# EricssonResearch/Robust-Tracking-MPC-over-Lossy-Networks

Hardware: AMD Instinct MI355X
Metric: QP solves/sec (= MPC steps/sec) at batch (higher is better)
Workload: dtype f64

## Files before the change

robust-tracking-mpc-over-lossy-networks_amd/csrc/tmpc_kernels.hip:

```cpp
#ifdef TMPC_HOST_SIM
#include "hip_sim.hpp"
#else
#include <hip/hip_runtime.h>
#endif

#include <algorithm>
#include <cmath>
#include <cstdint>
#include <string>
#include <type_traits>
#include <utility>

#include "tmpc_device.hpp"
#include "tmpc_launch.hpp"
#include "tmpc_wave.hpp"
#include "tmpc_mc_step.hpp"
#include "tmpc_law.hpp"
#include "tmpc_law_wave.hpp"

namespace tmpc {

namespace {

using wv::WAVE;
using wv::fast_rcp;
using wv::readlane_d;
using wv::lanes_backsub_lane;
using wv::lanes_factor;
using wv::lanes_forward;
using wv::vmax;
using wv::vmax_abs;
using wv::vmin;
using wv::OpMax;
using wv::OpMin;
using wv::OpSum;

constexpr int RED_STRIDE = 68;
constexpr int ZERO_ROWS = 4;

#if defined(TMPC_HOST_SIM)
#define STAMP(p) do { } while (0)
#elif defined(TMPC_STAMPS)
#define STAMP(p) do { asm volatile("s_waitcnt vmcnt(0) lgkmcnt(0)" ::: "memory"); long long now_ = __builtin_amdgcn_s_memtime(); \
                      asm volatile("s_waitcnt lgkmcnt(0)" ::: "memory"); tph[p] += now_ - tlast; tlast = now_; } while (0)
#else
#define STAMP(p) do { asm volatile("; MARK " #p); } while (0)
#endif

#ifndef TMPC_FENCE_ALL
#define TMPC_FENCE_ALL 0
#endif
#ifdef TMPC_HOST_SIM
__device__ __forceinline__ void row_fence() {}
__device__ __forceinline__ void wave_lds_fence() { sim::wave_fence(); }
#else
__device__ __forceinline__ void row_fence() {
    asm volatile("" ::: "memory");
    __builtin_amdgcn_sched_barrier(0);
}
__device__ __forceinline__ void wave_lds_fence() { asm volatile("" ::: "memory"); }
#endif

__device__ __forceinline__ double rcp1(double x) {
    const double r = __builtin_amdgcn_rcp(x);
    return fma(fma(-x, r, 1.0), r, r);
}

__device__ __forceinline__ double wave_sum(double v) { return wv::wave_reduce<OpSum>(v); }
__device__ __forceinline__ double wave_min(double v) { return wv::wave_reduce<OpMin>(v); }
__device__ __forceinline__ double wave_max(double v) { return wv::wave_reduce<OpMax>(v); }

__device__ __forceinline__ int fresh(int v) {
#ifdef TMPC_HOST_SIM
    asm volatile("" : "+r"(v));
#else
    asm volatile("" : "+v"(v));
#endif
    return v;
}

template <int N, class F>
__device__ __forceinline__ void static_for(F &&f) {
    [&]<int... I>(std::integer_sequence<int, I...>) { (f(std::integral_constant<int, I>{}), ...); }(std::make_integer_sequence<int, N>{});
}

template <class SH, int CNT>
__device__ __forceinline__ void wave_sums_to_lds(const double (&acc)[CNT], double *red, double *out, int lane) {
    static_assert(RED_STRIDE == wv::RED_STRIDE, "one tile layout");
    wv::swap_reduce_to_lds<CNT, SH::RR>(acc, red, out, lane);
}

template <class SH, int OFF, int CNT, int TOT>
__device__ __forceinline__ void wave_sums_part(const double (&acc)[TOT], double *red, double *out, int lane) {
    static_assert(OFF + CNT <= TOT, "part of the array");
    double part[CNT];
#pragma unroll
    for (int i = 0; i < CNT; ++i) part[i] = acc[OFF + i];
    wave_sums_to_lds<SH, CNT>(part, red, out, lane);
}
template <class SH, int CNT, int SPLIT>
__device__ __forceinline__ void wave_sums_to_lds2(const double (&acc)[CNT], double *red, double *out0, double *out1, int lane) {
    wv::swap_reduce_to_lds_at<CNT, SH::RR>(acc, red, [out0, out1](int e) { return e < SPLIT ? out0 + e : out1 + (e - SPLIT); }, lane);
}

template <class SH, int WPB>
constexpr bool sweep_b_one_round() { return SH::FD > 0 && SH::KC > 0 && !(WPB == 8 && SH::NV == 12); }

template <int NV>
__host__ __device__ constexpr int col_off(int j) { return j * NV - j * (j - 1) / 2; }

constexpr int tile_rows(int nv, int wpb) { return (wpb == 8 || nv > 24) ? 12 : 16; }

template <int NV_, int DP_, int DS_, int KC_, int CP_, int CS_, int RR_>
struct Shape {
    static constexpr int NV = NV_, DP = DP_, DS = DS_, KC = KC_, CP = CP_, CS = CS_, RR = RR_;
    static constexpr int KCA = KC_ > 0 ? KC_ : 1;
    static constexpr int FD = DP_ + DS_, FC = CP_ + CS_;
    static constexpr int NDP = FD * WAVE, NCCP = FC * WAVE;
    static constexpr int RS = 2 * DP_ + DS_ + 2 * CP_ + CS_;
    static constexpr bool SKIPS = NV_ == 11 && DP_ == 1 && DS_ == 0 && KC_ == 5 && CP_ == 4 && CS_ == 0;
    static constexpr int NT = NV_ * (NV_ + 1) / 2, KT = KC_ * (KC_ + 1) / 2;
    static constexpr int WCAP = NV_ <= 24 ? 24 : 28;
    static constexpr int odd_up(int v) { return v | 1; }
    static constexpr int LDH = odd_up(NV_);
    static constexpr int LDM = odd_up(NV_ + 1);
    static constexpr int LDW = odd_up(NV_), LDT = odd_up(WCAP);
    static constexpr int NB = (NV_ + 1 + 15) / 16;
    static constexpr int LDG = 16 * NB + 1;
    static constexpr int NTL = NB * (NB + 1) / 2;
    static constexpr int dbase(int kd) { return kd < DP_ ? 2 * kd : 2 * DP_ + (kd - DP_); }
    static constexpr int dsides(int kd) { return kd < DP_ ? 2 : 1; }
    static constexpr int cbase(int kc) { return 2 * DP_ + DS_ + (kc < CP_ ? 2 * kc : 2 * CP_ + (kc - CP_)); }
    static constexpr int csides(int kc) { return kc < CP_ ? 2 : 1; }
};

template <class SH>
__device__ __forceinline__ void side_info(int i, bool &dense, int &fslot, double &sgn) {
    if (i < 2 * SH::DP) { dense = true; fslot = i >> 1; sgn = (i & 1) ? -1.0 : 1.0; return; }
    if (i < 2 * SH::DP + SH::DS) { dense = true; fslot = SH::DP + (i - 2 * SH::DP); sgn = 1.0; return; }
    const int j = i - (2 * SH::DP + SH::DS);
    dense = false;
    if (j < 2 * SH::CP) { fslot = j >> 1; sgn = (j & 1) ? -1.0 : 1.0; return; }
    fslot = SH::CP + (j - 2 * SH::CP);
    sgn = 1.0;
}

template <class SH>
struct WaveLds {
    static constexpr int RED = SH::RR * RED_STRIDE;
    static constexpr int POL = SH::WCAP * SH::LDW + SH::NV * SH::LDT + 4 * SH::WCAP;
    static constexpr int MFAC = SH::NV * SH::LDM;
    static constexpr int BIG = RED + MFAC > POL ? RED + MFAC : POL;
    static constexpr int SUMS = 2 * SH::NV + 8;
    static constexpr int CSUMS = SH::KT + 2 * SH::KC + 8;
    static constexpr int PMAT = SH::KCA * SH::NV;
    static constexpr int HROW = SH::RS * WAVE;
    static constexpr int VEC = 9 * SH::NV + 32;
    static constexpr int TOTAL = BIG + SUMS + CSUMS + PMAT + HROW + VEC;
    static constexpr int PARK_WORDS = SH::RS * WAVE + 2;
    static constexpr int IDLE_WORDS = 2 * ((BIG - POL) + SUMS + CSUMS + PMAT);
#ifdef TMPC_PARK_HBM
    static constexpr bool PARK_LDS = false;
#else
    static constexpr bool PARK_LDS = IDLE_WORDS >= PARK_WORDS;
#endif
    static_assert(RED >= 2 * SH::NDP, "(D, t) of the dense functionals share the transposition tile");
};

template <class SH>
__device__ __forceinline__ void coords_lds(const double *Psi, const double *vec, double *out, int lane) {
    if constexpr (SH::KC > 0) {
        const int a_ = lane < SH::KC ? lane : 0;
        double t = 0.0;
#pragma unroll
        for (int j = 0; j < SH::NV; ++j) t += Psi[a_ * SH::NV + j] * vec[j];
        if (lane < SH::KC) out[lane] = t;
    }
}

template <class SH, int KD>
__device__ __forceinline__ double dense_dot(const double *Gt, int grows, const double *v, int lane) {
    const double *g = Gt + min(lane + KD * WAVE, grows) * SH::LDG;
    double t0 = 0.0, t1 = 0.0;
#pragma unroll
    for (int j = 0; j + 1 < SH::NV; j += 2) { t0 += g[j] * v[j]; t1 += g[j + 1] * v[j + 1]; }
    if (SH::NV & 1) t0 += g[SH::NV - 1] * v[SH::NV - 1];
    return t0 + t1;
}
template <class SH, int KCS>
__device__ __forceinline__ double fact_dot(const double *Hct, const double *c, int lane) {
    const int r = lane + KCS * WAVE;
    double t = 0.0;
#pragma unroll
    for (int a = 0; a < SH::KC; ++a) t += Hct[a * SH::NCCP + r] * c[a];
    return t;
}

typedef double v4d __attribute__((ext_vector_type(4)));
template <class SH>
__device__ __forceinline__ void sweep_a_dense(const double *Gt, int nks, const double (&s)[SH::RS], const double (&lam)[SH::RS],
                                              const double *rpw, double (&rs)[SH::RS], double &gap_l,
                                              double *dtw, double *mt, double *gdr, int lane) {
    constexpr int NV = SH::NV, NB = SH::NB, LDG = SH::LDG, IT = NV / 16, CT = NV % 16;
    static_for<SH::FD>([&](auto kd_) {
        constexpr int kd = decltype(kd_)::value;
        double D = 0.0, t = 0.0;
#pragma unroll
        for (int sd = 0; sd < SH::dsides(kd); ++sd) {
            constexpr int base = SH::dbase(kd);
            const int i = base + sd;
            const double rsi = fast_rcp(s[i]);
            rs[i] = rsi;
            const double d = lam[i] * rsi;
            const double rpi = rpw[i * WAVE + lane];
            gap_l = fma(s[i], lam[i], gap_l);
            D += d;
            t = sd ? fma(-d, rpi, t) : fma(d, rpi, t);
        }
        dtw[2 * (kd * WAVE + lane)] = D;
        dtw[2 * (kd * WAVE + lane) + 1] = t;
    });
    wave_lds_fence();
    const int c = lane & 15, kq = lane >> 4;
    const double tmask = (c == CT) ? 1.0 : 0.0;
    constexpr int NACC = SH::NTL == 1 ? 2 : 1;
    v4d acc[NACC][SH::NTL];
#pragma unroll
    for (int h2 = 0; h2 < NACC; ++h2)
#pragma unroll
        for (int q = 0; q < SH::NTL; ++q) acc[h2][q] = v4d{0.0, 0.0, 0.0, 0.0};
    const double *dp = dtw + 2 * kq, *gp = Gt + kq * LDG + c;
    auto fetch = [&](double &Dk, double &tk, double (&g)[NB]) {
        Dk = dp[0];
        tk = dp[1];
#pragma unroll
        for (int blk = 0; blk < NB; ++blk) g[blk] = gp[16 * blk];
        dp += 8;
        gp += 4 * LDG;
    };
    auto multiply = [&](auto h_, double Dk, double tk, const double (&g)[NB]) {
        constexpr int h2 = decltype(h_)::value;
        double a[NB];
#pragma unroll
        for (int blk = 0; blk < NB; ++blk) a[blk] = Dk * g[blk];
        a[IT] = fma(tmask, tk, a[IT]);
#pragma unroll
        for (int I = 0; I < NB; ++I)
#pragma unroll
            for (int J = 0; J <= I; ++J)
                acc[h2][I * (I + 1) / 2 + J] = __builtin_amdgcn_mfma_f64_16x16x4f64(a[I], g[J], acc[h2][I * (I + 1) / 2 + J], 0, 0, 0);
    };
    {
        double D0, t0, g0[NB], D1, t1, g1[NB];
        fetch(D0, t0, g0);
        int ks = 0;
        for (; ks + 1 < nks; ks += 2) {
            fetch(D1, t1, g1);
            multiply(std::integral_constant<int, 0>{}, D0, t0, g0);
            fetch(D0, t0, g0);
            multiply(std::integral_constant<int, NACC - 1>{}, D1, t1, g1);
        }
        if (ks < nks) multiply(std::integral_constant<int, 0>{}, D0, t0, g0);
    }
    static_assert(WaveLds<SH>::RED >= 2 * (SH::NDP + 4), "look-ahead of the MFMA pass stays inside the transposition tile");
    double *mtk = mt + kq * SH::LDM + c;
#pragma unroll
    for (int I = 0; I < NB; ++I)
#pragma unroll
        for (int J = 0; J <= I; ++J)
#pragma unroll
            for (int reg = 0; reg < 4; ++reg) {
                const int row = 16 * I + kq + 4 * reg, col = 16 * J + c;
                double v = acc[0][I * (I + 1) / 2 + J][reg];
                if constexpr (NACC == 2) v += acc[1][I * (I + 1) / 2 + J][reg];
                if (row < NV && col < NV) {
                    mtk[(16 * I + 4 * reg) * SH::LDM + 16 * J] = v;
                    if (I != J) mt[col * SH::LDM + row] = v;
                }
                if (I == IT && row == NV && col < NV) gdr[col] = v;
            }
    wave_lds_fence();
}

template <class SH, int NCS>
__device__ __forceinline__ void sweep_a_factored(const double *Hct, const double (&s)[SH::RS], const double (&lam)[SH::RS],
                                                 const double *rpw, double (&rs)[SH::RS], double &gap_l, double obj_l,
                                                 double *red, double *csums, int lane) {
    constexpr int KC = SH::KC, KT = SH::KT, NCCP = SH::NCCP;
    double acc[KT + KC + 2];
    static_for<NCS>([&](auto kc_) {
        constexpr int kc = decltype(kc_)::value;
        const int r = lane + kc * WAVE;
        double hc[KC];
#pragma unroll
        for (int a = 0; a < KC; ++a) hc[a] = Hct[a * NCCP + r];
        double D = 0.0, t = 0.0;
#pragma unroll
        for (int sd = 0; sd < SH::csides(kc); ++sd) {
            constexpr int base = SH::cbase(kc);
            const int i = base + sd;
            const double rsi = fast_rcp(s[i]);
            rs[i] = rsi;
            const double d = lam[i] * rsi;
            const double rpi = rpw[i * WAVE + lane];
            gap_l = fma(s[i], lam[i], gap_l);
            D += d;
            t = sd ? fma(-d, rpi, t) : fma(d, rpi, t);
        }
#pragma unroll
        for (int a = 0; a < KC; ++a) {
            const double dg = D * hc[a];
#pragma unroll
            for (int b2 = a; b2 < KC; ++b2) acc[col_off<KC>(a) + b2 - a] = kc == 0 ? dg * hc[b2] : fma(dg, hc[b2], acc[col_off<KC>(a) + b2 - a]);
            acc[KT + a] = kc == 0 ? hc[a] * t : fma(hc[a], t, acc[KT + a]);
        }
    });
    acc[KT + KC] = gap_l;
    acc[KT + KC + 1] = obj_l;
    wave_sums_to_lds<SH, KT + KC + 2>(acc, red, csums, lane);
}

struct McNone {};
struct McStepArg {
    const McFused *rec;
    int t;
    uint8_t *gamma_out;
};
struct McLawArg {
    const McFused *rec;
    const LawLoop *law;
};
template <int FUSED> using McArg = std::conditional_t<FUSED == 1, const McFused *, std::conditional_t<FUSED == 2, McStepArg, McNone>>;
template <int FUSED> using McBodyArg = std::conditional_t<FUSED == 3, McLawArg, McArg<FUSED>>;
#if defined(TMPC_HOST_SIM)
typedef const McFused *McRecord;
__device__ __forceinline__ McRecord mc_record(const McFused *p) { return p; }
#else
typedef const __attribute__((address_space(4))) McFused *McRecord;
__device__ __forceinline__ McRecord mc_record(const McFused *p) {
    unsigned lo = static_cast<unsigned>(reinterpret_cast<uintptr_t>(p)), hi = static_cast<unsigned>(reinterpret_cast<uintptr_t>(p) >> 32);
    asm volatile("" : "+v"(lo), "+v"(hi));
    lo = __builtin_amdgcn_readfirstlane(lo);
    hi = __builtin_amdgcn_readfirstlane(hi);
    return (McRecord)((static_cast<uintptr_t>(hi) << 32) | lo);
}
#endif
#if defined(TMPC_HOST_SIM)
typedef const LawLoop *LawRecord;
__device__ __forceinline__ LawRecord law_record(const LawLoop *p) { return p; }
#else
typedef const __attribute__((address_space(4))) LawLoop *LawRecord;
__device__ __forceinline__ LawRecord law_record(const LawLoop *p) {
    unsigned lo = static_cast<unsigned>(reinterpret_cast<uintptr_t>(p)), hi = static_cast<unsigned>(reinterpret_cast<uintptr_t>(p) >> 32);
    asm volatile("" : "+v"(lo), "+v"(hi));
    lo = __builtin_amdgcn_readfirstlane(lo);
    hi = __builtin_amdgcn_readfirstlane(hi);
    return (LawRecord)((static_cast<uintptr_t>(hi) << 32) | lo);
}
#endif

template <int NV, int DP, int DS, int KC, int CP, int CS, int WPB, int FUSED, int NCS>
__device__ __forceinline__ void solve_body(
    const DeviceQP &qp, const int variant_id, const int64_t B,
    const double *__restrict__ x_k, const double *__restrict__ ref, const uint8_t *__restrict__ variant,
    double *__restrict__ u_nom, double *__restrict__ x_nom0, double *__restrict__ xu_ss,
    double *__restrict__ x_nom, int32_t *__restrict__ status, int32_t *__restrict__ iters,
    const int32_t *ws_in, int32_t *ws_out, unsigned long long *__restrict__ next_item,
    const McBodyArg<FUSED> mc) {
    using SH = Shape<NV, DP, DS, KC, CP, CS, tile_rows(NV, WPB)>;
    using WL = WaveLds<SH>;
    constexpr int RS = SH::RS, FD = SH::FD, FC = SH::FC, NDP = SH::NDP, NCCP = SH::NCCP, KT = SH::KT, WCAP = SH::WCAP, LDG = SH::LDG;
#ifdef TMPC_HOST_SIM
    double *smem = sim::lds<double>();
#else
    extern __shared__ __attribute__((aligned(16))) double smem[];
#endif
    double *wbase = smem;
    double *Hct = wbase + WPB * WL::TOTAL;
    double *Psi = Hct + KC * NCCP;
    double *Hs = Psi + KC * NV;
    double *Hinv = Hs + NV * SH::LDH;
    double *Gt = Hinv + NV * SH::LDH;
    const int grows = 4 * qp.nks;

    const int tid = threadIdx.x;
    const int lane_k = tid & (WAVE - 1);
    int lane = lane_k;
    const int wave = __builtin_amdgcn_readfirstlane(tid >> 6);
    const int nx = qp.nx, nu = qp.nu, N = qp.N, nc = qp.nc;
    constexpr int RSL = NCS == FC ? RS : SH::cbase(NCS);
    static_assert(NCS == FC || (SH::SKIPS && NCS == FC - 1), "the slot counts a layout of this shape can have");

    for (int i = tid; i < (grows + ZERO_ROWS) * LDG; i += blockDim.x) Gt[i] = (i < grows * LDG) ? qp.Gt[i] : 0.0;
    for (int i = tid; i < KC * NCCP; i += blockDim.x) Hct[i] = qp.Hct[i];
    for (int i = tid; i < KC * NV; i += blockDim.x) Psi[i] = qp.Psi[i];
    for (int i = tid; i < NV * NV; i += blockDim.x) { const int r_ = i / NV, c_ = i - r_ * NV; Hs[r_ * SH::LDH + c_] = qp.Hs[i]; Hinv[r_ * SH::LDH + c_] = qp.Hinv[i]; }
    __syncthreads();

    double *red = wbase + wave * WL::TOTAL;
    double *sums = red + WL::BIG;
    double *csums = sums + WL::SUMS;
    double *Pm = csums + WL::CSUMS;
    double *hw = Pm + WL::PMAT;
    double *vec = hw + WL::HROW;
    double *dtw = red;
    double *Mf = red + WL::RED;
    unsigned *park = reinterpret_cast<unsigned *>(red + WL::POL);
    double *qv = vec;
    double *zv = vec + NV;
    double *cgv = vec + 2 * NV;
    double *xin = vec + 3 * NV;
    double *tv = vec + 3 * NV + 32;
    double *uv = vec + 4 * NV + 32;
    double *dzav = vec + 5 * NV + 32;
    double *dzv = vec + 6 * NV + 32;
    double *czv = vec + 7 * NV + 32;
    double *cdzav = czv + 8;
    double *cdzv = czv + 16;

    const int vmask_k = static_cast<int>(qp.vmask[lane]);
    unsigned vmask = static_cast<unsigned>(vmask_k);
    auto valid = [&](int i) { return ((vmask >> i) & 1u) != 0u; };
#define TMPC_REFRESH() do { lane = fresh(lane_k); vmask = static_cast<unsigned>(fresh(vmask_k)); } while (0)

    const int64_t n_waves = static_cast<int64_t>(gridDim.x) * WPB;
    bool first_item = true;
    for (;;) {
        int64_t b;
        if (first_item) {
            b = B < n_waves ? static_cast<int64_t>(wave) * gridDim.x + blockIdx.x : static_cast<int64_t>(blockIdx.x) * WPB + wave;
            first_item = false;
        } else {
            unsigned long long drawn = ~0ull >> 2;
            if (lane_k == 0) {
                const unsigned long long seen = __hip_atomic_load(next_item, __ATOMIC_RELAXED, __HIP_MEMORY_SCOPE_AGENT);
                if (n_waves + static_cast<int64_t>(seen) < B) drawn = atomicAdd(next_item, 1ull);
            }
            b = n_waves + static_cast<int64_t>((static_cast<unsigned long long>(static_cast<unsigned>(__builtin_amdgcn_readfirstlane(static_cast<int>(drawn >> 32)))) << 32) |
                                               static_cast<unsigned>(__builtin_amdgcn_readfirstlane(static_cast<int>(drawn & 0xffffffffull))));
        }
        if (b >= B) break;
        if (variant != nullptr && variant[b] != variant_id) continue;
        if (variant == nullptr && variant_id != 0) continue;

        int n_steps = 1;
        if constexpr (FUSED == 1) n_steps = mc_record(mc)->T;
        if constexpr (FUSED == 3) n_steps = mc_record(mc.rec)->T;
        for (int t_mc = 0; t_mc < n_steps; ++t_mc) {
        TMPC_REFRESH();
        if constexpr (FUSED != 0) {
            McRecord mr;
            if constexpr (FUSED == 1) mr = mc_record(mc); else mr = mc_record(mc.rec);
            const double *xh = mr->st.x_hat, *rk = mr->st.ref_k;
            if (lane < nx) { xin[lane] = xh[b * nx + lane]; xin[nx + lane] = rk[b * nx + lane]; }
        } else {
            if (lane < nx) { xin[lane] = x_k[b * nx + lane]; xin[nx + lane] = ref[b * nx + lane]; }
        }
        wave_lds_fence();
        bool law_hit = false;
        if constexpr (FUSED == 3) {
            const LawRecord lr = law_record(mc.law);
            const int np = 2 * nx;
            const bool finite = __ballot(lane < np && !law_finite(xin[lane < np ? lane : 0])) == 0ull;
            int32_t *const region = lr->region;
            int tried = 0, chain_tests = 0, chain_end = LAW_HOP_NONE;
            const int max_hops = lr->max_hops;
            const int win = finite ? law_find(&lr->t[0], np, xin, __builtin_amdgcn_readfirstlane(region[b]), lr->max_tries, lane, tried, max_hops,
                                              chain_tests, chain_end)
                                   : -1;
            if (lane == 0 && max_hops > 0) law_count_hops(lr->hop_stats, chain_tests, chain_end);
            if (win >= 0) {
                const int ny0 = N * nu, ny = ny0 + 2 * nx + nu;
                const double *Kt = lr->t[0].K;
                for (int j = lane; j < ny; j += WAVE) {
                    const double s = law_row(Kt, win, ny, np, xin, j);
                    if (j < ny0) u_nom[b * ny0 + j] = s;
                    else if (j < ny0 + nx) x_nom0[b * nx + (j - ny0)] = s;
                    else xu_ss[b * (nx + nu) + (j - ny0 - nx)] = s;
                }
                if (lane == 0) {
                    status[b] = TMPC_STATUS_OPTIMAL;
                    iters[b] = 0;
                    if (qp.ticks) qp.ticks[b] = 0;
                    region[b] = win;
                    lr->hits[b] += 1;
                    lr->tries[b] += tried;
                    unsigned long long *th = lr->t[0].hits;
                    if (th) atomicAdd(th + win, 1ull);
                }
                law_hit = true;
            } else {
                unsigned long long *mn = lr->miss_n;
                unsigned long long slot = 0;
                if (lane == 0) {
                    region[b] = -1;
                    lr->tries[b] += tried;
                    slot = atomicAdd(mn, 1ull);
                }
                const unsigned lo = static_cast<unsigned>(__builtin_amdgcn_readfirstlane(static_cast<int>(slot & 0xffffffffull)));
                const unsigned hi = static_cast<unsigned>(__builtin_amdgcn_readfirstlane(static_cast<int>(slot >> 32)));
                const long long at = static_cast<long long>((static_cast<unsigned long long>(hi) << 32) | lo);
                if (at < lr->miss_cap) {
                    if (lane < np) lr->miss_p[at * np + lane] = xin[lane];
                    if (lane == 0) lr->miss_var[at] = 0;
                }
            }
        }
        if (!law_hit) {
        int st = TMPC_STATUS_MAX_ITER;
        int it_done = 0;
#ifdef TMPC_ITERS_TOTAL
        int n_reruns = 0, n_rounds = 0, amb_level = 0;
#endif
        const long long t_begin = qp.ticks ? static_cast<long long>(__builtin_amdgcn_s_memrealtime()) : 0;
#ifdef TMPC_STAMPS
        long long tph[16] = {0, 0, 0, 0, 0, 0, 0, 0, 0, 0, 0, 0, 0, 0, 0, 0};
        long long tlast = __builtin_amdgcn_s_memtime();
#endif
        bool infeasible_par = qp.always_infeasible != 0;
        for (int r = lane; r < qp.npar; r += WAVE) {
            double v = qp.gp0[r];
            for (int c = 0; c < nx; ++c) v += qp.Ep[r * nx + c] * xin[c];
            if (v < -1e-9 * (1.0 + fabs(qp.gp0[r]))) infeasible_par = true;
        }
        infeasible_par = __any(infeasible_par);

        if (lane < NV) {
            double v = 0.0;
            if (lane < qp.nv)
                for (int c = 0; c < nx; ++c) v += qp.F1s[lane * nx + c] * xin[c] + qp.F2s[lane * nx + c] * xin[nx + c];
            qv[lane] = v;
        }
        auto compute_h = [&]() {
            TMPC_REFRESH();
            double hv[RS];
            const double *__restrict__ E0 = qp.Esp + lane;
            constexpr size_t PL = static_cast<size_t>(RS) * WAVE;
            for (int c0 = 0; c0 < nx; c0 += 4) {
                double ev[4][RS];
#pragma unroll
                for (int u = 0; u < 4; ++u) {
                    const size_t cu = static_cast<size_t>(c0 + u < nx ? c0 + u : nx - 1);
#pragma unroll
                    for (int i = 0; i < RSL; ++i) ev[u][i] = E0[cu * PL + i * WAVE];
                }
                if (c0 == 0) {
#pragma unroll
                    for (int i = 0; i < RSL; ++i) hv[i] = qp.g0p[i * WAVE + lane];
                }
#pragma unroll
                for (int u = 0; u < 4; ++u) {
                    const double xc = c0 + u < nx ? xin[c0 + u] : 0.0;
#pragma unroll
                    for (int i = 0; i < RSL; ++i) hv[i] = fma(ev[u][i], xc, hv[i]);
                }
            }
            double hmax = 1.0;
#pragma unroll
            for (int i = 0; i < RSL; ++i) {
                if (valid(i)) hmax = fmax(hmax, fabs(hv[i]));
                hw[i * WAVE + lane] = hv[i];
            }
            wave_lds_fence();
            return hmax;
        };
        const double hn = wave_max(compute_h());
        double qn = 1.0;
#pragma unroll
        for (int j = 0; j < NV; ++j) qn = fmax(qn, fabs(qv[j]));
        qn = readlane_d(qn, 0);

        auto unconstrained_minimiser = [&]() {
            TMPC_REFRESH();
            if (lane < NV) {
                double v = 0.0;
#pragma unroll
                for (int j = 0; j < NV; ++j) v -= Hinv[lane * SH::LDH + j] * qv[j];
                zv[lane] = v;
            }
            wave_lds_fence();
            coords_lds<SH>(Psi, zv, czv, lane);
            wave_lds_fence();
        };
        auto raw_slacks = [&](double (&sl)[RS]) {
            TMPC_REFRESH();
            double smin = INFINITY;
            static_for<FD>([&](auto kd_) {
                constexpr int kd = decltype(kd_)::value;
                const double gz = dense_dot<SH, kd>(Gt, grows, zv, lane);
#pragma unroll
                for (int sd = 0; sd < SH::dsides(kd); ++sd) {
                    const int i = SH::dbase(kd) + sd;
                    sl[i] = hw[i * WAVE + lane] - (sd ? -gz : gz);
                    if (valid(i)) smin = vmin(smin, sl[i]);
                }
            });
            static_for<NCS>([&](auto kc_) {
                constexpr int kc = decltype(kc_)::value;
                const double gz = fact_dot<SH, kc>(Hct, czv, lane);
#pragma unroll
                for (int sd = 0; sd < SH::csides(kc); ++sd) {
                    const int i = SH::cbase(kc) + sd;
                    sl[i] = hw[i * WAVE + lane] - (sd ? -gz : gz);
                    if (valid(i)) smin = vmin(smin, sl[i]);
                }
            });
#pragma unroll
            for (int i = RSL; i < RS; ++i) sl[i] = 1.0;
            return smin;
        };

        double try_tol = qp.tol;
        const double ncd = static_cast<double>(nc);
        double rdn_last = 0.0;
        bool floor_tried = false;
        bool inW[RS];
        double yall[RS];
        int warm_m = 0;
        {
            unconstrained_minimiser();
            double sl[RS];
            const double smin = wave_min(raw_slacks(sl));
            if (infeasible_par) st = TMPC_STATUS_INFEASIBLE;
            else if (smin >= 0.0) st = TMPC_STATUS_OPTIMAL;
            if (ws_in != nullptr) warm_m = ws_in[b * WS_STRIDE];
        }
        STAMP(0);
        bool try_warm = warm_m > 0 && warm_m <= WCAP;
        int resume_it = -1;
        float *const save = qp.save ? qp.save + (static_cast<size_t>(blockIdx.x) * WPB + wave) * (2 * RS * WAVE) : nullptr;
        bool saved = false;
        bool h_valid = true;
        int ws_m = 0;
        if (st == TMPC_STATUS_MAX_ITER)
        for (;;) {
            bool want_polish = false;
            if (try_warm) {
#pragma unroll
                for (int i = 0; i < RS; ++i) { inW[i] = false; yall[i] = 0.0; }
                for (int k = 0; k < warm_m; ++k) {
                    const int gid = ws_in[b * WS_STRIDE + 1 + k];
#pragma unroll
                    for (int i = 0; i < RS; ++i) inW[i] = inW[i] || (gid == i * WAVE + lane && valid(i));
                }
                want_polish = true;
            } else {
                double s[RS], lam[RS], rs[RS];
                double *rpw = hw;
                double kappa = 1.0, rpn0 = 0.0;
                int it0 = 0;
                double mu_hand = 0.0;
                if (resume_it >= 0) {
                    if (!h_valid) { compute_h(); h_valid = true; }
                    coords_lds<SH>(Psi, zv, czv, lane);
                    wave_lds_fence();
                    (void)raw_slacks(s);
                    h_valid = false;
                    const double park_mu = WL::PARK_LDS ? *reinterpret_cast<const double *>(park + RS * WAVE) : 0.0;
                    const double park_thr = 1e3 * try_tol * hn;
#pragma unroll
                    for (int i = 0; i < RSL; ++i) {
                        const bool vl = valid(i);
                        const double raw = s[i];
                        double sv, lv;
                        if constexpr (WL::PARK_LDS) {
                            lv = fmax(static_cast<double>(__uint_as_float(park[i * WAVE + lane])), 1e-30);
                            sv = raw > park_thr ? raw : fmin(fmax(raw, park_mu * fast_rcp(lv)), park_thr);
                        } else {
                            sv = static_cast<double>(save[i * WAVE + lane]);
                            lv = static_cast<double>(save[(RS + i) * WAVE + lane]);
                            if (raw > 0.0 && fabs(sv - raw) <= 2.5e-7 * sv) sv = raw;
                        }
                        s[i] = vl ? sv : 1.0;
                        lam[i] = vl ? lv : 0.0;
                        const double rp0 = vl ? sv - raw : 0.0;
                        rpw[i * WAVE + lane] = rp0;
                        rpn0 = vmax_abs(rpn0, rp0);
                        rs[i] = 1.0;
                    }
#pragma unroll
                    for (int i = RSL; i < RS; ++i) { s[i] = 1.0; lam[i] = 0.0; rs[i] = 1.0; }
                    wave_lds_fence();
                    it0 = resume_it;
                    resume_it = -1;
                } else {
                    if (!h_valid) { compute_h(); h_valid = true; }
                    unconstrained_minimiser();
                    const double smin = wave_min(raw_slacks(s));
                    const double fl = 0.1 * fmax(-smin, 1.0);
                    h_valid = false;
                    double l1 = 0.0;
#pragma unroll
                    for (int i = 0; i < RSL; ++i) l1 = vmax(l1, valid(i) ? -s[i] * qp.cip[i * WAVE + lane] : 0.0);
                    l1 = wave_max(l1);
#ifdef TMPC_LAM0_ONE
                    const double lam0 = l1 < 0.0 ? 2.0 : 1.0;
#else
                    const double lam0 = fmin(fmax(sqrt(sqrt(l1)), 1.0), 1e3);
#endif
// ... 965 lines not shown
```

robust-tracking-mpc-over-lossy-networks_amd/csrc/tmpc_wave.hpp:

```cpp
#pragma once
#ifdef TMPC_HOST_SIM
#include "hip_sim.hpp"
#else
#include <hip/hip_runtime.h>
#endif

#include <utility>

namespace tmpc {
namespace wv {

constexpr int WAVE = 64;

__device__ __forceinline__ double fast_rcp(double x) {
    double r = __builtin_amdgcn_rcp(x);
    r = fma(fma(-x, r, 1.0), r, r);
    r = fma(fma(-x, r, 1.0), r, r);
    return r;
}

template <int CTRL>
__device__ __forceinline__ double dpp_mov_d(double v) {
    int lo = __double2loint(v), hi = __double2hiint(v);
    lo = __builtin_amdgcn_update_dpp(lo, lo, CTRL, 0xF, 0xF, false);
    hi = __builtin_amdgcn_update_dpp(hi, hi, CTRL, 0xF, 0xF, false);
    return __hiloint2double(hi, lo);
}
__device__ __forceinline__ double readlane_d(double v, int l) {
    const int lo = __builtin_amdgcn_readlane(__double2loint(v), l);
    const int hi = __builtin_amdgcn_readlane(__double2hiint(v), l);
    return __hiloint2double(hi, lo);
}
#ifdef TMPC_HOST_SIM
__device__ __forceinline__ double vmax(double a, double b) { return fmax(a, b); }
__device__ __forceinline__ double vmin(double a, double b) { return fmin(a, b); }
__device__ __forceinline__ double vmax_abs(double a, double b) { return fmax(a, fabs(b)); }
#else
__device__ __forceinline__ double vmax(double a, double b) {
    double r;
    asm("v_max_f64 %0, %1, %2" : "=v"(r) : "v"(a), "v"(b));
    return r;
}
__device__ __forceinline__ double vmin(double a, double b) {
    double r;
    asm("v_min_f64 %0, %1, %2" : "=v"(r) : "v"(a), "v"(b));
    return r;
}
__device__ __forceinline__ double vmax_abs(double a, double b) {
    double r;
    asm("v_max_f64 %0, %1, |%2|" : "=v"(r) : "v"(a), "v"(b));
    return r;
}
#endif
struct OpSum { __device__ __forceinline__ static double f(double a, double b) { return a + b; } };
struct OpMin { __device__ __forceinline__ static double f(double a, double b) { return vmin(a, b); } };
struct OpMax { __device__ __forceinline__ static double f(double a, double b) { return vmax(a, b); } };

template <class Op>
__device__ __forceinline__ double wave_reduce(double v) {
    v = Op::f(v, dpp_mov_d<0xB1>(v));
    v = Op::f(v, dpp_mov_d<0x4E>(v));
    v = Op::f(v, dpp_mov_d<0x141>(v));
    v = Op::f(v, dpp_mov_d<0x140>(v));
    const double r0 = readlane_d(v, 0), r1 = readlane_d(v, 16), r2 = readlane_d(v, 32), r3 = readlane_d(v, 48);
    return Op::f(Op::f(r0, r1), Op::f(r2, r3));
}

#ifdef TMPC_HOST_SIM
__device__ __forceinline__ void lds_fence() { sim::wave_fence(); }
#else
__device__ __forceinline__ void lds_fence() { asm volatile("" ::: "memory"); }
#endif

constexpr int RED_STRIDE = 68;
template <int CNT>
__device__ __forceinline__ void reduce_to_lds(const double (&acc)[CNT], double *red, double *out, int lane) {
    const int e = lane >> 2, qd = lane & 3;
    const int wcol = lane + (lane >> 4);
#pragma unroll
    for (int c0 = 0; c0 < CNT; c0 += 16) {
#pragma unroll
        for (int k = 0; k < 16; ++k)
            if (c0 + k < CNT) red[k * RED_STRIDE + wcol] = acc[c0 + k];
        lds_fence();
        double t = 0.0;
#pragma unroll
        for (int j = 0; j < 16; ++j) t += red[e * RED_STRIDE + qd * 17 + j];
        t += dpp_mov_d<0xB1>(t);
        t += dpp_mov_d<0x4E>(t);
        if (qd == 0 && c0 + e < CNT) out[c0 + e] = t;
        lds_fence();
    }
}

template <int HALF>
__device__ __forceinline__ void permlane_swap(int &x, int &y, int lane) {
    static_assert(HALF == 32 || HALF == 16, "v_permlane32_swap / v_permlane16_swap");
#ifdef TMPC_HOST_SIM
    const int xo = __builtin_amdgcn_readlane(x, lane ^ HALF), yo = __builtin_amdgcn_readlane(y, lane ^ HALF);
    const bool up = (lane & HALF) != 0;
    x = up ? yo : x;
    y = up ? y : xo;
#else
    (void)lane;
    if constexpr (HALF == 32) {
        const auto r = __builtin_amdgcn_permlane32_swap(x, y, false, false);
        x = static_cast<int>(r[0]);
        y = static_cast<int>(r[1]);
    } else {
        const auto r = __builtin_amdgcn_permlane16_swap(x, y, false, false);
        x = static_cast<int>(r[0]);
        y = static_cast<int>(r[1]);
    }
#endif
}
template <int HALF>
__device__ __forceinline__ double swap_add(double a, double b, int lane) {
    int alo = __double2loint(a), ahi = __double2hiint(a), blo = __double2loint(b), bhi = __double2hiint(b);
    permlane_swap<HALF>(alo, blo, lane);
    permlane_swap<HALF>(ahi, bhi, lane);
    return __hiloint2double(ahi, alo) + __hiloint2double(bhi, blo);
}

__device__ __forceinline__ void wave_sum2(double &a, double &b, int lane) {
    double v = swap_add<32>(a, b, lane);
    v += dpp_mov_d<0xB1>(v);
    v += dpp_mov_d<0x4E>(v);
    v += dpp_mov_d<0x141>(v);
    v += dpp_mov_d<0x140>(v);
    a = readlane_d(v, 0) + readlane_d(v, 16);
    b = readlane_d(v, 32) + readlane_d(v, 48);
}

template <int CNT, int RR, class OutAt>
__device__ __forceinline__ void swap_reduce_to_lds_at(const double (&acc)[CNT], double *red, OutAt &&out_at, int lane) {
    constexpr int H1 = (CNT + 1) / 2, H2 = (H1 + 1) / 2;
    double r1[H1];
#pragma unroll
    for (int c = 0; c < H1; ++c) r1[c] = swap_add<32>(acc[c], c + H1 < CNT ? acc[c + H1] : 0.0, lane);
    double r2[H2];
#pragma unroll
    for (int d = 0; d < H2; ++d) r2[d] = swap_add<16>(r1[d], d + H2 < H1 ? r1[d + H2] : 0.0, lane);
    auto entry = [](int d, int r) {
        const int e = d + (r & 1) * H2 + (r >> 1) * H1;
        return ((r & 1) && d + H2 >= H1) || e >= CNT ? -1 : e;
    };
    const int wcol = lane + (lane >> 4);
    const int k = lane >> 2, qd = lane & 3;
#pragma unroll
    for (int d0 = 0; d0 < H2; d0 += RR) {
#pragma unroll
        for (int d = 0; d < RR; ++d)
            if (d0 + d < H2) red[d * RED_STRIDE + wcol] = r2[d0 + d];
        lds_fence();
        constexpr int NR = RR < 16 ? RR : 16;
        const int kr = k < NR && d0 + k < H2 ? k : 0;
        double t4[4] = {0.0, 0.0, 0.0, 0.0};
#pragma unroll
        for (int j = 0; j < 16; ++j) t4[j & 3] += red[kr * RED_STRIDE + qd * 17 + j];
        const double t = (t4[0] + t4[1]) + (t4[2] + t4[3]);
        const int e = (k < NR && d0 + k < H2) ? entry(d0 + k, qd) : -1;
        if (e >= 0) *out_at(e) = t;
        lds_fence();
    }
}
template <int CNT, int RR>
__device__ __forceinline__ void swap_reduce_to_lds(const double (&acc)[CNT], double *red, double *out, int lane) {
    swap_reduce_to_lds_at<CNT, RR>(acc, red, [out](int e) { return out + e; }, lane);
}

template <int N>
__device__ __forceinline__ bool rows_factor(double (&row)[N], double &b, double &dinv, int lane) {
    bool ok = true;
#pragma unroll
    for (int k = 0; k < N; ++k) {
        const double pkk = readlane_d(row[k], k);
        ok = ok && (pkk > 0.0);
        const double pinv = fast_rcp(pkk);
        const double f = (lane > k) ? row[k] * pinv : 0.0;
#pragma unroll
        for (int j = k + 1; j < N; ++j) row[j] = fma(-f, readlane_d(row[j], k), row[j]);
        b = fma(-f, readlane_d(b, k), b);
        if (lane > k) row[k] = f;
        if (lane == k) dinv = pinv;
    }
    return ok;
}
template <int N>
__device__ __forceinline__ void rows_forward(const double (&row)[N], double &b, int lane) {
#pragma unroll
    for (int k = 0; k < N - 1; ++k) {
        const double f = (lane > k) ? row[k] : 0.0;
        b = fma(-f, readlane_d(b, k), b);
    }
}
template <int N>
__device__ __forceinline__ double rows_backsub_lane(const double (&row)[N], double b, double dinv, int lane) {
    double xl = 0.0;
#pragma unroll
    for (int i = N - 1; i >= 0; --i) {
        const double bi = b * dinv;
        const double xi = readlane_d(bi, i);
        xl = (lane == i) ? bi : xl;
        b = fma(-row[i], xi, b);
    }
    return xl;
}

template <int K>
__device__ __forceinline__ double row_bcast_d(double v) {
    return __builtin_amdgcn_mov_dpp(v, 0x150 + K, 0xF, 0xF, false);
}
template <int N, class F>
__device__ __forceinline__ void static_for_n(F &&f) {
    [&]<int... I>(std::integer_sequence<int, I...>) { (f(std::integral_constant<int, I>{}), ...); }(std::make_integer_sequence<int, N>{});
}
template <int K, int NOPS>
__device__ __forceinline__ void fmac_bcast(double &acc, double v, double m) {
#if defined(TMPC_HOST_SIM) || defined(TMPC_NO_DPP_FMAC)
    acc = fma(row_bcast_d<K>(v), m, acc);
#else
    if constexpr (NOPS > 0)
        asm volatile("s_nop %3\n\tv_fmac_f64_dpp %0, %1, %2 row_newbcast:%4 row_mask:0xf bank_mask:0xf"
                     : "+v"(acc) : "v"(v), "v"(m), "n"(NOPS - 1), "n"(K));
    else
        asm volatile("v_fmac_f64_dpp %0, %1, %2 row_newbcast:%3 row_mask:0xf bank_mask:0xf" : "+v"(acc) : "v"(v), "v"(m), "n"(K));
#endif
}
template <int K, int NOPS>
__device__ __forceinline__ double row_bcast_ordered(double v) {
#if defined(TMPC_HOST_SIM) || defined(TMPC_NO_DPP_FMAC)
    return row_bcast_d<K>(v);
#else
    double r;
    if constexpr (NOPS > 0)
        asm volatile("s_nop %2\n\tv_mov_b64_dpp %0, %1 row_newbcast:%3 row_mask:0xf bank_mask:0xf" : "=v"(r) : "v"(v), "n"(NOPS - 1), "n"(K));
    else
        asm volatile("v_mov_b64_dpp %0, %1 row_newbcast:%2 row_mask:0xf bank_mask:0xf" : "=v"(r) : "v"(v), "n"(K));
    return r;
#endif
}
__device__ __forceinline__ void pin(double &v) {
#if !defined(TMPC_HOST_SIM) && !defined(TMPC_NO_DPP_FMAC)
    asm volatile("" : "+v"(v));
#endif
}
template <int N>
__device__ __forceinline__ bool rows16_factor(double (&row)[N], double &b, double &dinv, int lane) {
    static_assert(N <= 16, "one matrix row per lane of a 16-lane DPP row");
    const int l16 = lane & 15;
    bool ok = true;
    pin(b);
    double pkk = row_bcast_ordered<0, 0>(row[0]);
    double pinv = fast_rcp(pkk);
    static_for_n<N>([&](auto k_) {
        constexpr int k = decltype(k_)::value;
        ok = ok && (pkk > 0.0);
        const double pinv_k = pinv;
        const double f = (l16 > k) ? row[k] * pinv_k : 0.0;
        const double nf = -f;
        constexpr int NU = N - 1 - k;
        static_for_n<(NU < 3 ? NU : 3)>([&](auto j_) {
            constexpr int j = k + 1 + decltype(j_)::value;
            fmac_bcast<k, 0>(row[j], row[j], nf);
        });
        if constexpr (NU < 3) fmac_bcast<k, 0>(b, b, nf);
        if constexpr (k + 1 < N) {
            pkk = row_bcast_ordered<k + 1, (NU == 1 ? 2 : 0)>(row[k + 1]);
            pinv = fast_rcp(pkk);
        }
        if constexpr (NU >= 3) {
            static_for_n<NU - 3>([&](auto j_) {
                constexpr int j = k + 4 + decltype(j_)::value;
                fmac_bcast<k, 0>(row[j], row[j], nf);
            });
            fmac_bcast<k, 0>(b, b, nf);
        }
        if (l16 > k) row[k] = f;
        if (l16 == k) dinv = pinv_k;
    });
    return __builtin_amdgcn_readfirstlane(static_cast<int>(ok)) != 0;
}
template <int N>
__device__ __forceinline__ void rows16_forward(const double (&row)[N], double &b, int lane) {
    const int l16 = lane & 15;
    static_for_n<N - 1>([&](auto k_) {
        constexpr int k = decltype(k_)::value;
        const double f = (l16 > k) ? row[k] : 0.0;
        b = fma(-f, row_bcast_d<k>(b), b);
    });
}
template <int N>
__device__ __forceinline__ double rows16_backsub_lane(const double (&row)[N], double b, double dinv, int lane) {
    const int l16 = lane & 15;
    double xl = 0.0;
    static_for_n<N>([&](auto r_) {
        constexpr int i = N - 1 - decltype(r_)::value;
        const double bi = b * dinv;
        const double xi = row_bcast_d<i>(bi);
        xl = (l16 == i) ? bi : xl;
        b = fma(-row[i], xi, b);
    });
    return xl;
}
template <int N, int LDM>
__device__ __forceinline__ bool rows32_factor_solve(double *Mf, const double *rhs, double *x, int lane) {
    static_assert(N > 16 && N <= 32, "two matrix rows per lane");
    const int l16 = lane & 15;
    const bool hasb = l16 + 16 < N;
    const int ib = hasb ? l16 + 16 : 0;
    double ra[N], rb[N];
#pragma unroll
    for (int j = 0; j < N; ++j) { ra[j] = Mf[l16 * LDM + j]; rb[j] = Mf[ib * LDM + j]; }
    double ba = rhs[l16], bb = hasb ? rhs[ib] : 0.0;
    double da = 1.0, db = 1.0;
    lds_fence();
    bool ok = true;
    pin(ba);
    pin(bb);
    static_for_n<N>([&](auto k_) {
        constexpr int k = decltype(k_)::value;
        constexpr bool inA = k < 16;
        constexpr int kl = k & 15;
        double pkk;
        if constexpr (inA) pkk = row_bcast_ordered<kl, (k >= N - 2 ? 2 : 0)>(ra[k]);
        else pkk = row_bcast_ordered<kl, (k >= N - 2 ? 2 : 0)>(rb[k]);
        ok = ok && (pkk > 0.0);
        const double pinv = fast_rcp(pkk);
        double nfa = 0.0;
        if constexpr (inA) nfa = (l16 > k) ? -ra[k] * pinv : 0.0;
        const double nfb = (hasb && l16 + 16 > k) ? -rb[k] * pinv : 0.0;
        static_for_n<N - 1 - k>([&](auto j_) {
            constexpr int j = k + 1 + decltype(j_)::value;
            if constexpr (inA) {
                fmac_bcast<kl, 0>(rb[j], ra[j], nfb);
                fmac_bcast<kl, 0>(ra[j], ra[j], nfa);
            } else {
                fmac_bcast<kl, 0>(rb[j], rb[j], nfb);
            }
        });
        if constexpr (inA) {
            fmac_bcast<kl, 0>(bb, ba, nfb);
            fmac_bcast<kl, 0>(ba, ba, nfa);
            if (l16 > k) ra[k] = -nfa;
            if (l16 == k) da = pinv;
        } else {
            fmac_bcast<kl, 0>(bb, bb, nfb);
            if (l16 == kl) db = pinv;
        }
        if (hasb && l16 + 16 > k) rb[k] = -nfb;
    });
    ok = __builtin_amdgcn_readfirstlane(static_cast<int>(ok)) != 0;
    if (!ok) return false;
    double xa = 0.0, xb = 0.0;
    static_for_n<N>([&](auto r_) {
        constexpr int i = N - 1 - decltype(r_)::value;
        constexpr int il = i & 15;
        if constexpr (i >= 16) {
            const double bi = bb * db;
            const double xi = row_bcast_d<il>(bi);
            xb = (l16 == il) ? bi : xb;
            bb = fma(-rb[i], xi, bb);
            ba = fma(-ra[i], xi, ba);
        } else {
            const double bi = ba * da;
            const double xi = row_bcast_d<il>(bi);
            xa = (l16 == il) ? bi : xa;
            ba = fma(-ra[i], xi, ba);
        }
    });
    if (lane < 16) {
        x[l16] = xa;
        if (hasb) x[ib] = xb;
#pragma unroll
        for (int j = 0; j < N; ++j) Mf[l16 * LDM + j] = ra[j];
        Mf[l16 * LDM + N] = da;
        if (hasb) {
#pragma unroll
            for (int j = 0; j < N; ++j) Mf[ib * LDM + j] = rb[j];
            Mf[ib * LDM + N] = db;
        }
    }
    lds_fence();
    return true;
}
template <int N, int LDM>
__device__ __forceinline__ void rows32_resolve(const double *Mf, const double *rhs, double *x, int lane) {
    const int l16 = lane & 15;
    const bool hasb = l16 + 16 < N;
    const int ib = hasb ? l16 + 16 : 0;
    double ra[N], rb[N];
#pragma unroll
    for (int j = 0; j < N; ++j) { ra[j] = Mf[l16 * LDM + j]; rb[j] = Mf[ib * LDM + j]; }
    const double da = Mf[l16 * LDM + N], db = Mf[ib * LDM + N];
    double ba = rhs[l16], bb = hasb ? rhs[ib] : 0.0;
    lds_fence();
    static_for_n<N - 1>([&](auto k_) {
        constexpr int k = decltype(k_)::value;
        constexpr int kl = k & 15;
        const double fb = (hasb && l16 + 16 > k) ? rb[k] : 0.0;
        if constexpr (k < 16) {
            const double fa = (l16 > k) ? ra[k] : 0.0;
            const double xk = row_bcast_d<kl>(ba);
            ba = fma(-fa, xk, ba);
            bb = fma(-fb, xk, bb);
        } else {
            const double xk = row_bcast_d<kl>(bb);
            bb = fma(-fb, xk, bb);
        }
    });
    double xa = 0.0, xb = 0.0;
    static_for_n<N>([&](auto r_) {
        constexpr int i = N - 1 - decltype(r_)::value;
        constexpr int il = i & 15;
        if constexpr (i >= 16) {
            const double bi = bb * db;
            const double xi = row_bcast_d<il>(bi);
            xb = (l16 == il) ? bi : xb;
            bb = fma(-rb[i], xi, bb);
            ba = fma(-ra[i], xi, ba);
        } else {
            const double bi = ba * da;
            const double xi = row_bcast_d<il>(bi);
            xa = (l16 == il) ? bi : xa;
            ba = fma(-ra[i], xi, ba);
        }
    });
    if (lane < 16) {
        x[l16] = xa;
        if (hasb) x[ib] = xb;
    }
    lds_fence();
}

#ifdef TMPC_NO_DPP64
constexpr int DPP_ROW = 0;
#else
constexpr int DPP_ROW = 16;
#endif
template <int N>
__device__ __forceinline__ bool lanes_factor(double (&row)[N], double &b, double &dinv, int lane) {
    if constexpr (N <= DPP_ROW) return rows16_factor<N>(row, b, dinv, lane);
    else return rows_factor<N>(row, b, dinv, lane);
}
template <int N>
__device__ __forceinline__ void lanes_forward(const double (&row)[N], double &b, int lane) {
    if constexpr (N <= DPP_ROW) rows16_forward<N>(row, b, lane);
    else rows_forward<N>(row, b, lane);
}
template <int N>
__device__ __forceinline__ double lanes_backsub_lane(const double (&row)[N], double b, double dinv, int lane) {
    if constexpr (N <= DPP_ROW) return rows16_backsub_lane<N>(row, b, dinv, lane);
    else return rows_backsub_lane<N>(row, b, dinv, lane);
}

}
}
```

Baseline: 12.88 million.

## Use 4x4x4 f64 MFMA block tiles for small G'DG assembly and batch staging loads

```diff
diff --git a/robust-tracking-mpc-over-lossy-networks_amd/csrc/tmpc_kernels.hip b/robust-tracking-mpc-over-lossy-networks_amd/csrc/tmpc_kernels.hip
--- a/robust-tracking-mpc-over-lossy-networks_amd/csrc/tmpc_kernels.hip
+++ b/robust-tracking-mpc-over-lossy-networks_amd/csrc/tmpc_kernels.hip
@@ -128,6 +128,11 @@
     static constexpr int NB = (NV_ + 1 + 15) / 16;
     static constexpr int LDG = 16 * NB + 1;
     static constexpr int NTL = NB * (NB + 1) / 2;
+#ifdef TMPC_NO_MFMA_BLOCKS
+    static constexpr bool MFMA_BLOCKS = false;
+#else
+    static constexpr bool MFMA_BLOCKS = NV_ <= 12 && KC_ > 0;
+#endif
     static constexpr int dbase(int kd) { return kd < DP_ ? 2 * kd : 2 * DP_ + (kd - DP_); }
     static constexpr int dsides(int kd) { return kd < DP_ ? 2 : 1; }
     static constexpr int cbase(int kc) { return 2 * DP_ + DS_ + (kc < CP_ ? 2 * kc : 2 * CP_ + (kc - CP_)); }
@@ -221,6 +226,11 @@
         dtw[2 * (kd * WAVE + lane) + 1] = t;
     });
     wave_lds_fence();
+    static_assert(WaveLds<SH>::RED >= 2 * (SH::NDP + 4), "look-ahead of the MFMA pass stays inside the transposition tile");
+    if constexpr (SH::MFMA_BLOCKS) {
+        wv::gdg_blocks<NV, LDG, SH::LDM>(Gt, nks, dtw, mt, gdr, lane);
+        return;
+    }
     const int c = lane & 15, kq = lane >> 4;
     const double tmask = (c == CT) ? 1.0 : 0.0;
     constexpr int NACC = SH::NTL == 1 ? 2 : 1;
@@ -262,7 +272,6 @@
         }
         if (ks < nks) multiply(std::integral_constant<int, 0>{}, D0, t0, g0);
     }
-    static_assert(WaveLds<SH>::RED >= 2 * (SH::NDP + 4), "look-ahead of the MFMA pass stays inside the transposition tile");
     double *mtk = mt + kq * SH::LDM + c;
 #pragma unroll
     for (int I = 0; I < NB; ++I)
@@ -391,10 +400,32 @@
     constexpr int RSL = NCS == FC ? RS : SH::cbase(NCS);
     static_assert(NCS == FC || (SH::SKIPS && NCS == FC - 1), "the slot counts a layout of this shape can have");
 
-    for (int i = tid; i < (grows + ZERO_ROWS) * LDG; i += blockDim.x) Gt[i] = (i < grows * LDG) ? qp.Gt[i] : 0.0;
-    for (int i = tid; i < KC * NCCP; i += blockDim.x) Hct[i] = qp.Hct[i];
-    for (int i = tid; i < KC * NV; i += blockDim.x) Psi[i] = qp.Psi[i];
-    for (int i = tid; i < NV * NV; i += blockDim.x) { const int r_ = i / NV, c_ = i - r_ * NV; Hs[r_ * SH::LDH + c_] = qp.Hs[i]; Hinv[r_ * SH::LDH + c_] = qp.Hinv[i]; }
+    {
+        constexpr int NT = WAVE * WPB;
+        constexpr int TG = ((NDP + ZERO_ROWS) * LDG + NT - 1) / NT, TH = (KC * NCCP + NT - 1) / NT, TP = (KC * NV + NT - 1) / NT, TS = (NV * NV + NT - 1) / NT;
+        const int ng = grows * LDG, nz = (grows + ZERO_ROWS) * LDG;
+        double vg[TG > 0 ? TG : 1], vh[TH > 0 ? TH : 1], vp[TP > 0 ? TP : 1], vs[TS], vi[TS];
+#pragma unroll
+        for (int u = 0; u < TG; ++u) { const int i = tid + u * NT; vg[u] = i < ng ? qp.Gt[i] : 0.0; }
+#pragma unroll
+        for (int u = 0; u < TH; ++u) { const int i = tid + u * NT; vh[u] = i < KC * NCCP ? qp.Hct[i] : 0.0; }
+#pragma unroll
+        for (int u = 0; u < TP; ++u) { const int i = tid + u * NT; vp[u] = i < KC * NV ? qp.Psi[i] : 0.0; }
+#pragma unroll
+        for (int u = 0; u < TS; ++u) { const int i = tid + u * NT; vs[u] = i < NV * NV ? qp.Hs[i] : 0.0; vi[u] = i < NV * NV ? qp.Hinv[i] : 0.0; }
+#pragma unroll
+        for (int u = 0; u < TG; ++u) { const int i = tid + u * NT; if (i < nz) Gt[i] = (SH::MFMA_BLOCKS && i < ng && i % LDG == NV) ? 1.0 : vg[u]; }
+        for (int i = tid + TG * NT; i < nz; i += NT) Gt[i] = i < ng ? qp.Gt[i] : 0.0;
+#pragma unroll
+        for (int u = 0; u < TH; ++u) { const int i = tid + u * NT; if (i < KC * NCCP) Hct[i] = vh[u]; }
+#pragma unroll
+        for (int u = 0; u < TP; ++u) { const int i = tid + u * NT; if (i < KC * NV) Psi[i] = vp[u]; }
+#pragma unroll
+        for (int u = 0; u < TS; ++u) {
+            const int i = tid + u * NT, r_ = i / NV, c_ = i - r_ * NV;
+            if (i < NV * NV) { Hs[r_ * SH::LDH + c_] = vs[u]; Hinv[r_ * SH::LDH + c_] = vi[u]; }
+        }
+    }
     __syncthreads();
 
     double *red = wbase + wave * WL::TOTAL;
diff --git a/robust-tracking-mpc-over-lossy-networks_amd/csrc/tmpc_wave.hpp b/robust-tracking-mpc-over-lossy-networks_amd/csrc/tmpc_wave.hpp
--- a/robust-tracking-mpc-over-lossy-networks_amd/csrc/tmpc_wave.hpp
+++ b/robust-tracking-mpc-over-lossy-networks_amd/csrc/tmpc_wave.hpp
@@ -5,6 +5,7 @@
 #include <hip/hip_runtime.h>
 #endif
 
+#include <cstdint>
 #include <utility>
 
 namespace tmpc {
@@ -454,5 +455,140 @@
     else return rows_backsub_lane<N>(row, b, dinv, lane);
 }
 
-}
-}
+constexpr int mb_block(int lane) { return (lane >> 2) & 3; }
+constexpr int mb_minor(int lane) { return lane & 3; }
+constexpr int mb_major(int lane) { return lane >> 4; }
+__device__ __forceinline__ double mfma_blocks(double a, double b, double c) {
+#ifdef TMPC_HOST_SIM
+    sim::Slot s{};
+    s.d[0] = a;
+    s.d[1] = b;
+    const sim::Slot *all = sim::wave_meet(sim::OP_MFMA, s);
+    const int l = sim::cur_lane(), base = 4 * mb_block(l), i = mb_major(l), j = mb_minor(l);
+    double acc = c;
+    for (int k = 0; k < 4; ++k) acc = std::fma(all[16 * k + base + i].d[0], all[16 * k + base + j].d[1], acc);
+    return acc;
+#else
+    return __builtin_amdgcn_mfma_f64_4x4x4f64(a, b, c, 0, 0, 0);
+#endif
+}
+
+#ifdef TMPC_HOST_SIM
+typedef const double *lds_cptr;
+__device__ __forceinline__ lds_cptr lds_opaque(const double *p) { return p; }
+#else
+typedef const __attribute__((address_space(3))) double *lds_cptr;
+__device__ __forceinline__ lds_cptr lds_opaque(const double *p) {
+    unsigned a = static_cast<unsigned>(reinterpret_cast<uintptr_t>((lds_cptr)p));
+    asm("" : "+v"(a));
+    return reinterpret_cast<lds_cptr>(static_cast<uintptr_t>(a));
+}
+#endif
+template <int NV>
+struct GdgBlocks {
+    static constexpr int NBR = (NV + 1 + 3) / 4, NBC = (NV + 3) / 4;
+    static constexpr int first(int I) { return I <= NBC ? I * (I + 1) / 2 : NBC * (NBC + 1) / 2 + (I - NBC) * NBC; }
+    static constexpr int NBLK = first(NBR);
+    static constexpr int NI = (NBLK + 3) / 4;
+    static constexpr int brow(int q) { int I = 0; while (first(I + 1) <= q) ++I; return I; }
+    static constexpr int bcol(int q) { return q - first(brow(q)); }
+    static constexpr int slotq(int n, int bs) { return NBLK - 4 * (NI - n) + bs; }
+    static constexpr int clampq(int q) { return q < 0 ? 0 : q; }
+    static constexpr bool takes_t(int n) { return brow(clampq(slotq(n, 3))) == NV / 4; }
+    static constexpr bool any_plain() { for (int n = 0; n < NI; ++n) if (!takes_t(n)) return true; return false; }
+};
+template <int NV, int LDG, int LDM>
+__device__ __forceinline__ void gdg_blocks(const double *Gt, int nks, const double *dtw, double *mt, double *gdr, int lane) {
+    using GB = GdgBlocks<NV>;
+    constexpr int NI = GB::NI;
+    static_assert(4 * GB::NBR <= LDG, "the rows of the last block row read columns of G that are staged");
+    const int kq = mb_major(lane), bs = mb_block(lane), r = mb_minor(lane);
+    int r0[NI], c0[NI];
+    static_for_n<NI>([&](auto n_) {
+        constexpr int n = decltype(n_)::value;
+        constexpr int q0 = GB::clampq(GB::slotq(n, 0)), q1 = GB::clampq(GB::slotq(n, 1)), q2 = GB::clampq(GB::slotq(n, 2)), q3 = GB::clampq(GB::slotq(n, 3));
+        r0[n] = 4 * (bs == 0 ? GB::brow(q0) : bs == 1 ? GB::brow(q1) : bs == 2 ? GB::brow(q2) : GB::brow(q3));
+        c0[n] = 4 * (bs == 0 ? GB::bcol(q0) : bs == 1 ? GB::bcol(q1) : bs == 2 ? GB::bcol(q2) : GB::bcol(q3));
+    });
+    double acc[2][NI];
+#pragma unroll
+    for (int h2 = 0; h2 < 2; ++h2)
+#pragma unroll
+        for (int n = 0; n < NI; ++n) acc[h2][n] = 0.0;
+    lds_cptr pd = lds_opaque(dtw + 2 * kq), px[NI], pa[NI], pb[NI];
+#pragma unroll
+    for (int n = 0; n < NI; ++n) {
+        px[n] = GB::takes_t(n) ? lds_opaque(dtw + 2 * kq + (r0[n] + r == NV ? 1 : 0)) : pd;
+        pa[n] = lds_opaque(Gt + kq * LDG + r + r0[n]);
+        pb[n] = lds_opaque(Gt + kq * LDG + r + c0[n]);
+    }
+    struct Ops { double D, x[NI], ga[NI], gb[NI]; };
+    auto fetch = [&](Ops &o, auto u_) {
+        constexpr int u = decltype(u_)::value;
+        if constexpr (GB::any_plain()) o.D = pd[8 * u];
+#pragma unroll
+        for (int n = 0; n < NI; ++n) {
+            if (GB::takes_t(n)) o.x[n] = px[n][8 * u];
+            o.ga[n] = pa[n][4 * LDG * u];
+            o.gb[n] = pb[n][4 * LDG * u];
+        }
+    };
+    auto bump = [&](auto u_) {
+        constexpr int u = decltype(u_)::value;
+        pd += 8 * u;
+#pragma unroll
+        for (int n = 0; n < NI; ++n) { px[n] += 8 * u; pa[n] += 4 * LDG * u; pb[n] += 4 * LDG * u; }
+    };
+    auto multiply = [&](auto h_, const Ops &o) {
+        constexpr int h2 = decltype(h_)::value;
+        static_for_n<NI>([&](auto n_) {
+            constexpr int n = decltype(n_)::value;
+            const double a = (GB::takes_t(n) ? o.x[n] : o.D) * o.ga[n];
+            acc[h2][n] = mfma_blocks(a, o.gb[n], acc[h2][n]);
+        });
+    };
+    constexpr std::integral_constant<int, 0> c_0{};
+    constexpr std::integral_constant<int, 1> c_1{};
+    constexpr std::integral_constant<int, 2> c_2{};
+    constexpr std::integral_constant<int, 3> c_3{};
+    constexpr std::integral_constant<int, 4> c_4{};
+    {
+        Ops o0, o1;
+        fetch(o0, c_0);
+        int ks = 0;
+        for (; ks + 3 < nks; ks += 4) {
+            fetch(o1, c_1);
+            multiply(c_0, o0);
+            fetch(o0, c_2);
+            multiply(c_1, o1);
+            fetch(o1, c_3);
+            multiply(c_0, o0);
+            bump(c_4);
+            fetch(o0, c_0);
+            multiply(c_1, o1);
+        }
+        if (ks + 1 < nks) {
+            fetch(o1, c_1);
+            multiply(c_0, o0);
+            fetch(o0, c_2);
+            multiply(c_1, o1);
+            ks += 2;
+        }
+        if (ks < nks) multiply(c_0, o0);
+    }
+    static_for_n<NI>([&](auto n_) {
+        constexpr int n = decltype(n_)::value;
+        const double v = acc[0][n] + acc[1][n];
+        const int row = r0[n] + kq, col = c0[n] + r;
+        const bool mine = GB::slotq(n, 0) + bs >= 0;
+        if (mine && row < NV && col <= row) {
+            mt[row * LDM + col] = v;
+            if (col < row) mt[col * LDM + row] = v;
+        }
+        if (mine && row == NV && col < NV) gdr[col] = v;
+    });
+    lds_fence();
+}
+
+}
+}
```

Measured after the change: 13.02 million, median of 6. 1.0% higher.
